# frederik-kofoed-marqversen/quantum_computations

Hardware: AMD Instinct MI355X
Metric: gate_apps_per_sec (higher is better)
Workload: dtype f64; 1 GPU; 28-qubit complex128 state vector (28 qubits = 4 GiB per GPU), depth-100 random 1+2-qubit gates (BASELINE.json configs[1], seed 100); n_qubits=28

## Files before the change

### quantum_computations_amd/build.py

```python
from __future__ import annotations

import os
import shutil
import subprocess
import sys
from pathlib import Path

PKG_DIR = Path(__file__).resolve().parent
REPO_ROOT = PKG_DIR.parent
CSRC = PKG_DIR / "csrc"
LIB_PATH = PKG_DIR / "libqsv.so"
SOURCES = ["qsv_api.hip", "qsv_kernels.hip", "qsv_qudit.hip", "qsv_gemm.hip", "qsv_decomp.hip", "qsv_circuit.hip",
           "qsv_phase_space.hip", "qsv_sampling.hip", "qsv_canonical.hip"]
HEADERS = [CSRC / "qsv_internal.h", CSRC / "qsv_linalg.h", CSRC / "qsv_plan.h", CSRC / "qsv_layout.h", CSRC / "qsv_pauli_plan.h",
           CSRC / "qsv_pauli_rotation_plan.h", REPO_ROOT / "include" / "qsv.h"]
ARCH = "gfx950"


def hipcc() -> str:
    for cand in (os.environ.get("HIPCC"), shutil.which("hipcc"), "/opt/rocm/bin/hipcc"):
        if cand and Path(cand).exists():
            return cand
    raise RuntimeError("hipcc not found: libqsv.so needs the ROCm toolchain (there is no CPU fallback)")


def _stale(target: Path, deps: list[Path]) -> bool:
    if not target.exists():
        return True
    t = target.stat().st_mtime
    return any(d.stat().st_mtime > t for d in deps)


def build_lib(force: bool = False, verbose: bool = False) -> Path:
    objs = []
    build_dir = PKG_DIR / "build"
    build_dir.mkdir(exist_ok=True)
    flags = [f"--offload-arch={ARCH}", "-O3", "-std=c++17", "-fPIC", "-Wall", "-Wno-unused-function",
             f"-I{REPO_ROOT / 'include'}", f"-I{CSRC}"]
    for name in SOURCES:
        src = CSRC / name
        obj = build_dir / (name + ".o")
        if force or _stale(obj, [src] + HEADERS):
            cmd = [hipcc(), *flags, "-c", str(src), "-o", str(obj)]
            if verbose:
                print(" ".join(cmd), flush=True)
            subprocess.run(cmd, check=True)
        objs.append(obj)
    if force or _stale(LIB_PATH, objs):
        cmd = [hipcc(), f"--offload-arch={ARCH}", "-shared", "-fPIC", "-o", str(LIB_PATH), *map(str, objs), "-ldl"]
        if verbose:
            print(" ".join(cmd), flush=True)
        subprocess.run(cmd, check=True)
    return LIB_PATH


if __name__ == "__main__":
    path = build_lib(force="--force" in sys.argv, verbose=True)
    print(path)
```

### quantum_computations_amd/csrc/qsv_kernels.hip

```cpp

#include "qsv_internal.h"
#include "qsv_layout.h"
#include "qsv_plan.h"

#include <algorithm>
#include <array>
#include <cstdlib>
#include <cstring>
#include <type_traits>
#include <vector>

using namespace qsv_layout;
static_assert(LANE_BITS == QSV_LANE_BITS && MAX_K == QSV_MAX_K && BLOCK == QSV_BLOCK, "qsv_layout.h and qsv_internal.h agree");

namespace {

struct cplx {
    double re, im;
};

__device__ __forceinline__ amp_t cmul(cplx m, amp_t a) {
    amp_t r;
    r.x = m.re * a.x - m.im * a.y;
    r.y = m.re * a.y + m.im * a.x;
    return r;
}

__device__ __forceinline__ amp_t cmul_diag(cplx d, amp_t a) {
    amp_t r;
    r.x = fma(a.x, d.re, -(a.y * d.im));
    r.y = fma(a.x, d.im, a.y * d.re);
    return r;
}

__device__ __forceinline__ amp_t cfma(cplx m, amp_t a, amp_t acc) {
    amp_t r;
    r.x = fma(m.re, a.x, fma(-m.im, a.y, acc.x));
    r.y = fma(m.re, a.y, fma(m.im, a.x, acc.y));
    return r;
}

template <bool NT>
__device__ __forceinline__ amp_t ld(const amp_t *p) {
    if constexpr (NT)
        return __builtin_nontemporal_load(p);
    else
        return *p;
}

template <bool NT>
__device__ __forceinline__ void st(amp_t *p, amp_t v) {
    if constexpr (NT)
        __builtin_nontemporal_store(v, p);
    else
        *p = v;
}

__device__ __forceinline__ amp_t shfl_xor_amp(amp_t v, int lane_mask) {
    amp_t r;
    r.x = __shfl_xor(v.x, lane_mask, 64);
    r.y = __shfl_xor(v.y, lane_mask, 64);
    return r;
}

__device__ __forceinline__ uint64_t insert_zero(uint64_t w, int p) {
    const uint64_t low = w & ((1ull << p) - 1ull);
    return ((w >> p) << (p + 1)) | low;
}

template <class Args>
__device__ __forceinline__ uint64_t deposit(uint64_t w, const Args &g) {
    for (int j = 0; j < g.nins; ++j) w = insert_zero(w, static_cast<int>(g.pos[j]));
    return w | g.or_mask;
}

template <int KH, int KL, int U, bool NT>
__device__ __forceinline__ void dense_body(amp_t *__restrict__ a, const GateArgs &g) {
    constexpr int NH = 1 << KH, NL = 1 << KL, D = NH * NL;
    const int lane = threadIdx.x & 63;
    const bool lane_ok = (static_cast<uint32_t>(lane) & g.lane_ctrl) == g.lane_ctrl;

    int l = 0;
#pragma unroll
    for (int j = 0; j < KL; ++j) l |= ((lane >> g.lbit[j]) & 1) << j;

    cplx coef[NH][NH][NL];
#pragma unroll
    for (int h = 0; h < NH; ++h)
#pragma unroll
        for (int hp = 0; hp < NH; ++hp)
#pragma unroll
            for (int x = 0; x < NL; ++x) {
// ... 2188 lines not shown
    return rc ? rc : qsvk_stage_done(st, staged);
}

int qsvk_sequence_tile(qsv_state *st, int k, const int *bits, int n_gates, const int *arity, const int *legs,
                       const double *mats) {
    if (k < 1 || k > 6 || n_gates < 1 || n_gates > SEQ_MAX_GATES || st->n < TILE_SEQ_BITS) return QSV_UNHANDLED_KQ;
    const TileCut cut = cut_tile_passes(st->n, k, bits, n_gates, arity, legs, mats);
    if (cut.status == TileCut::UNHANDLED) return QSV_UNHANDLED_KQ;
    if (cut.status == TileCut::LEG_OUTSIDE) return qsv_fail(QSV_EINVAL, "gate sequence: leg outside the block");
    if (cut.status == TileCut::LEGS_EQUAL) return qsv_fail(QSV_EINVAL, "gate sequence: legs outside the block");
    const std::vector<int> &tile_bits = cut.tile_bits;
    const std::vector<uint64_t> off = offsets(std::vector<int>(tile_bits.begin() + 6, tile_bits.end()));
    const size_t gates_bytes = qsv_pad16(sizeof(SeqGate) * cut.rec.size()), passes_bytes = qsv_pad16(sizeof(TilePass) * cut.passes.size());
    std::vector<char> image(gates_bytes + passes_bytes, 0);
    std::memcpy(image.data(), cut.rec.data(), sizeof(SeqGate) * cut.rec.size());
    std::memcpy(image.data() + gates_bytes, cut.passes.data(), sizeof(TilePass) * cut.passes.size());
    StageRef staged;
    int rc = qsvk_stage(st, image.data(), image.size(), off.data(), sizeof(uint64_t) * off.size(), &staged);
    if (rc) return rc;
    const SeqGate *dev_g = reinterpret_cast<const SeqGate *>(staged.dev);
    const TilePass *dev_p = reinterpret_cast<const TilePass *>(staged.dev + gates_bytes);
    const uint64_t *dev_off = reinterpret_cast<const uint64_t *>(staged.dev + qsv_pad16(image.size()));
    TileSeqArgs ta;
    std::memset(&ta, 0, sizeof(ta));
    ta.g = with_enumeration<BigArgs>(enumeration(st->amps >> TILE_SEQ_BITS, tile_bits));
    for (int j = 0; j < 6; ++j) ta.lane_bit[j] = static_cast<uint32_t>(tile_bits[j]);
    ta.g.regions = regions_or(st, 8);
    const bool nt = st->nontemporal != 0;
    const size_t lds = sizeof(amp_t) << TILE_SEQ_BITS;
    static bool raised = false;
    if (!raised) {
        QSV_HIP(hipFuncSetAttribute(reinterpret_cast<const void *>(k_seq_tile<true>), hipFuncAttributeMaxDynamicSharedMemorySize,
                                    static_cast<int>(lds)));
        QSV_HIP(hipFuncSetAttribute(reinterpret_cast<const void *>(k_seq_tile<false>), hipFuncAttributeMaxDynamicSharedMemorySize,
                                    static_cast<int>(lds)));
        raised = true;
    }
    snprintf(st->last_kernel, sizeof(st->last_kernel), "k_seq_tile<%s>", nt ? "true" : "false");
    const int n_passes = static_cast<int>(cut.passes.size());
    st->last_passes = n_passes;
    rc = launch_ranges(ta.g, DISPATCH_TILES, [&](uint64_t tiles) {
        const dim3 gd(static_cast<unsigned>(tiles)), bd(TILE_SEQ_THREADS);
        with_bool(nt, [&](auto NT) { hipLaunchKernelGGL(k_seq_tile<NT.value>, gd, bd, lds, st->stream, st->data, ta, dev_g, dev_p, n_passes, dev_off); });
    });
    return rc ? rc : qsvk_stage_done(st, staged);
}

constexpr int PASS_TILE = 1 << qsv_plan::TILE_BITS, PASS_ROWS = PASS_TILE / 64, PASS_THREADS = 256;
constexpr int PASS_ROWS_PER_WAVE = PASS_ROWS / (PASS_THREADS / 64);
static_assert(PASS_TILE == PASS_THREADS << qsv_plan::REG_BITS, "one thread per setting of the tile bits outside the registers");

struct PassArgs {
    BigArgs g;
    uint64_t row_off[PASS_ROWS];
};

template <int FORM>
__device__ __forceinline__ constexpr int pass_col(int r, int j) {
    return FORM == 0 ? j : FORM == 1 ? (j ^ r) : (((j & 1) << 1) | ((r & 1) ^ (j >> 1)));
}

struct PassCtl {
    uint32_t rc;
    bool sel;
    bool ok;
};

__device__ __forceinline__ void pass_put(amp_t &x, amp_t y, const PassCtl &ct) {
    if (ct.sel) {
        x.x = ct.ok ? y.x : x.x;
        x.y = ct.ok ? y.y : x.y;
    } else {
        x = y;
    }
}

template <int D, int FORM, int P0, int P1>
__device__ __forceinline__ void pass_dense(amp_t (&x)[16], const double *__restrict__ m, const PassCtl &ct) {
    constexpr int TARGETS = (1 << P0) | (D == 4 ? (1 << P1) : 0);
#pragma unroll
    for (int b = 0; b < 16; ++b) {
        if (b & TARGETS) continue;
        if ((b & ct.rc) != ct.rc) continue;
        int idx[D];
#pragma unroll
        for (int c = 0; c < D; ++c) idx[c] = b | ((c & 1) << P0) | (D == 4 ? ((c >> 1) << P1) : 0);
        amp_t y[D];
#pragma unroll
        for (int r = 0; r < D; ++r) {
            amp_t acc = {0.0, 0.0};
#pragma unroll
            for (int j = 0; j < D; ++j) {
                const int c = pass_col<FORM>(r, j);
                acc = cfma(cplx{m[2 * (r * D + c)], m[2 * (r * D + c) + 1]}, x[idx[c]], acc);
            }
            y[r] = acc;
        }
#pragma unroll
        for (int r = 0; r < D; ++r) pass_put(x[idx[r]], y[r], ct);
    }
}

template <int PA, int PB>
__device__ __forceinline__ void pass_pair(amp_t (&x)[16], const PassCtl &ct) {
#pragma unroll
    for (int b = 0; b < 16; ++b) {
        if (b & ((1 << PA) | (1 << PB))) continue;
        if ((b & ct.rc) != ct.rc) continue;
        const amp_t u = x[b | (1 << PA)], v = x[b | (1 << PB)];
        pass_put(x[b | (1 << PA)], v, ct);
        pass_put(x[b | (1 << PB)], u, ct);
    }
}

template <class Sel>
__device__ __forceinline__ void pass_diag(amp_t (&x)[16], const cplx (&d)[4], const PassCtl &ct, Sel sel) {
#pragma unroll
    for (int c = 0; c < 16; ++c) {
        if ((c & ct.rc) != ct.rc) continue;
        pass_put(x[c], cmul_diag(d[sel(c)], x[c]), ct);
    }
}

__device__ __forceinline__ cplx pass_pick(bool s, cplx one, cplx zero) {
    return cplx{s ? one.re : zero.re, s ? one.im : zero.im};
}

__device__ __forceinline__ void pass_gate16(amp_t (&x)[16], const PassGate &pg, uint32_t g0) {
    const double *__restrict__ m = pg.m;
    const PassCtl ct = {pg.rc, pg.tc != 0, (g0 & pg.tc) == pg.tc};
#define QSV_PASS_D4(FORM, P0, P1) case (FORM) * 16 + (P0) * 4 + (P1): pass_dense<4, (FORM) - PASS_D4, P0, P1>(x, m, ct); break;
#define QSV_PASS_D4_BOTH(FORM, LO, HI) QSV_PASS_D4(FORM, LO, HI) QSV_PASS_D4(FORM, HI, LO)
    switch (pg.form * 16 + pg.code) {
        case PASS_D2 * 16 + 0: pass_dense<2, 0, 0, 0>(x, m, ct); break;
        case PASS_D2 * 16 + 1: pass_dense<2, 0, 1, 0>(x, m, ct); break;
        case PASS_D2 * 16 + 2: pass_dense<2, 0, 2, 0>(x, m, ct); break;
        case PASS_D2 * 16 + 3: pass_dense<2, 0, 3, 0>(x, m, ct); break;
        case PASS_D2X * 16 + 0: pass_dense<2, 1, 0, 0>(x, m, ct); break;
        case PASS_D2X * 16 + 1: pass_dense<2, 1, 1, 0>(x, m, ct); break;
        case PASS_D2X * 16 + 2: pass_dense<2, 1, 2, 0>(x, m, ct); break;
        case PASS_D2X * 16 + 3: pass_dense<2, 1, 3, 0>(x, m, ct); break;
        QSV_PASS_D4_BOTH(PASS_D4, 0, 1) QSV_PASS_D4_BOTH(PASS_D4, 0, 2) QSV_PASS_D4_BOTH(PASS_D4, 0, 3)
        QSV_PASS_D4_BOTH(PASS_D4, 1, 2) QSV_PASS_D4_BOTH(PASS_D4, 1, 3) QSV_PASS_D4_BOTH(PASS_D4, 2, 3)
        QSV_PASS_D4_BOTH(PASS_D4X, 0, 1) QSV_PASS_D4_BOTH(PASS_D4X, 0, 2) QSV_PASS_D4_BOTH(PASS_D4X, 0, 3)
        QSV_PASS_D4_BOTH(PASS_D4X, 1, 2) QSV_PASS_D4_BOTH(PASS_D4X, 1, 3) QSV_PASS_D4_BOTH(PASS_D4X, 2, 3)
        QSV_PASS_D4(PASS_D4HL, 0, 1) QSV_PASS_D4(PASS_D4HL, 0, 2) QSV_PASS_D4(PASS_D4HL, 0, 3)
        QSV_PASS_D4(PASS_D4HL, 1, 2) QSV_PASS_D4(PASS_D4HL, 1, 3) QSV_PASS_D4(PASS_D4HL, 2, 3)
        case PASS_PAIR * 16 + 0 * 4 + 1: pass_pair<0, 1>(x, ct); break;
        case PASS_PAIR * 16 + 0 * 4 + 2: pass_pair<0, 2>(x, ct); break;
        case PASS_PAIR * 16 + 0 * 4 + 3: pass_pair<0, 3>(x, ct); break;
        case PASS_PAIR * 16 + 1 * 4 + 2: pass_pair<1, 2>(x, ct); break;
        case PASS_PAIR * 16 + 1 * 4 + 3: pass_pair<1, 3>(x, ct); break;
        case PASS_PAIR * 16 + 2 * 4 + 3: pass_pair<2, 3>(x, ct); break;
        case PASS_DIAG_T * 16: {
            const bool s0 = (g0 >> pg.tz0) & 1, s1 = (g0 >> pg.tz1) & 1;
            const cplx d[4] = {pass_pick(s0, pass_pick(s1, cplx{m[6], m[7]}, cplx{m[4], m[5]}),
                                         pass_pick(s1, cplx{m[2], m[3]}, cplx{m[0], m[1]})), {}, {}, {}};
            pass_diag(x, d, ct, [](int) { return 0; });
            break;
        }
#define QSV_PASS_R1(P) case PASS_DIAG_R1 * 16 + (P): { \
            const cplx d[4] = {{m[0], m[1]}, {m[2], m[3]}, {}, {}}; \
            pass_diag(x, d, ct, [](int c) { return (c >> (P)) & 1; }); break; }
        QSV_PASS_R1(0) QSV_PASS_R1(1) QSV_PASS_R1(2) QSV_PASS_R1(3)
#define QSV_PASS_R2(P0, P1) case PASS_DIAG_R2 * 16 + (P0) * 4 + (P1): { \
            const cplx d[4] = {{m[0], m[1]}, {m[2], m[3]}, {m[4], m[5]}, {m[6], m[7]}}; \
            pass_diag(x, d, ct, [](int c) { return (((c >> (P0)) & 1) << 1) | ((c >> (P1)) & 1); }); break; }
        QSV_PASS_R2(0, 1) QSV_PASS_R2(0, 2) QSV_PASS_R2(0, 3) QSV_PASS_R2(1, 2) QSV_PASS_R2(1, 3) QSV_PASS_R2(2, 3)
#define QSV_PASS_M(P) case PASS_DIAG_M * 16 + (P): { \
            const bool s = (g0 >> pg.tz0) & 1; \
            const cplx d[4] = {pass_pick(s, cplx{m[2], m[3]}, cplx{m[0], m[1]}), pass_pick(s, cplx{m[6], m[7]}, cplx{m[4], m[5]}), {}, {}}; \
            pass_diag(x, d, ct, [](int c) { return (c >> (P)) & 1; }); break; }
        QSV_PASS_M(0) QSV_PASS_M(1) QSV_PASS_M(2) QSV_PASS_M(3)
        default: break;
    }
#undef QSV_PASS_D4
#undef QSV_PASS_D4_BOTH
#undef QSV_PASS_R1
#undef QSV_PASS_R2
#undef QSV_PASS_M
}

template <bool NT>
__global__ __launch_bounds__(PASS_THREADS) void k_pass_tile(amp_t *__restrict__ a, const PassArgs pa,
                                                            const PassGate *__restrict__ gates, int n_gates,
                                                            const PassGroup *__restrict__ groups, int n_groups) {
    __shared__ amp_t tile[PASS_TILE];
    const BigArgs &g = pa.g;
    const int lane = threadIdx.x & 63;
    const int q = __builtin_amdgcn_readfirstlane(threadIdx.x >> 6);
    constexpr int RPW = PASS_ROWS_PER_WAVE;
    const uint64_t tile_id = (g.regions > 1 && gridDim.x % g.regions == 0)
                                 ? (blockIdx.x % g.regions) * (gridDim.x / g.regions) + blockIdx.x / g.regions
                                 : blockIdx.x;
    const uint64_t base = deposit(g.w0 + tile_id, g);
    uint64_t active = 0;
    for (int i = 0; i < n_gates; ++i)
        if ((base & gates[i].omask) == gates[i].omask) active |= 1ull << i;
    if (!active) return;
#if defined(__HIP_DEVICE_COMPILE__)
#pragma unroll
    for (int i = 0; i < RPW; ++i)
        __builtin_amdgcn_global_load_lds(a + base + pa.row_off[q * RPW + i] + lane, tile + (q * RPW + i) * 64, 16, 0, NT ? 2 : 0);
#endif
    __syncthreads();
#pragma unroll 1
    for (int p = 0; p < n_groups; ++p) {
        const PassGroup &gr = groups[p];
        if (!(active & gr.gates)) continue;
        const int q0 = gr.q[0], q1 = gr.q[1], q2 = gr.q[2], q3 = gr.q[3];
        uint32_t g0 = threadIdx.x;
        g0 = static_cast<uint32_t>(insert_zero(g0, q0));
        g0 = static_cast<uint32_t>(insert_zero(g0, q1));
        g0 = static_cast<uint32_t>(insert_zero(g0, q2));
        g0 = static_cast<uint32_t>(insert_zero(g0, q3));
        amp_t x[16];
#pragma unroll
        for (int c = 0; c < 16; ++c)
            x[c] = tile[g0 | ((c & 1) << q0) | (((c >> 1) & 1) << q1) | (((c >> 2) & 1) << q2) | (((c >> 3) & 1) << q3)];
#pragma unroll 1
        for (int i = gr.first; i < gr.first + gr.count; ++i)
            if ((active >> i) & 1) pass_gate16(x, gates[i], g0);
#pragma unroll
        for (int c = 0; c < 16; ++c)
            tile[g0 | ((c & 1) << q0) | (((c >> 1) & 1) << q1) | (((c >> 2) & 1) << q2) | (((c >> 3) & 1) << q3)] = x[c];
        __syncthreads();
    }
#pragma unroll
    for (int i = 0; i < RPW; ++i) st<NT>(a + base + pa.row_off[q * RPW + i] + lane, tile[(q * RPW + i) * 64 + lane]);
}

bool qsvk_op_exact(const QsvOp &op) {
    if (op.kind == QSV_OP_PAIR) return true;
    auto unit = [](double re, double im) { return im == 0.0 && (re == 1.0 || re == -1.0); };
    if (op.kind == QSV_OP_PHASE) return unit(op.m[0], op.m[1]);
    if (op.kind == QSV_OP_DIAG) {
        for (int i = 0; i < (1 << op.k); ++i)
            if (!unit(op.m[2 * i], op.m[2 * i + 1])) return false;
        return true;
    }
    const int D = 1 << op.k;
    int per_col[4] = {0, 0, 0, 0};
    for (int r = 0; r < D; ++r) {
        int nz = 0;
        for (int c = 0; c < D; ++c) {
            const double re = op.m[2 * (r * D + c)], im = op.m[2 * (r * D + c) + 1];
            if (re == 0.0 && im == 0.0) continue;
            if (!unit(re, im)) return false;
            ++nz;
            ++per_col[c];
        }
        if (nz != 1) return false;
    }
    for (int c = 0; c < D; ++c)
        if (per_col[c] != 1) return false;
    return true;
}

int qsvk_run_op(qsv_state *st, const QsvOp &op) {
    switch (op.kind) {
        case QSV_OP_DENSE: return qsvk_dense(st, op.k, op.bits, op.nctrl, op.cbits, op.m);
        case QSV_OP_PAIR: return qsvk_pair_exchange(st, op.bits[0], op.bits[1]);
        case QSV_OP_DIAG: return qsvk_diag(st, op.k, op.bits, op.nctrl, op.cbits, op.m);
        case QSV_OP_PHASE: return qsvk_phase(st, op.nctrl, op.cbits, op.m[0], op.m[1]);
        default: return qsv_fail(QSV_EINVAL, "internal: unknown queued gate kind");
    }
}

int qsvk_pass(qsv_state *st, const QsvOp *const *ops, int count, uint64_t tile_high) {
    const uint64_t low = (1ull << QSV_LANE_BITS) - 1;
    if (count < 1 || count > qsv_plan::MAX_PASS_GATES || st->n < qsv_plan::TILE_BITS || (tile_high & low) ||
        __builtin_popcountll(tile_high) != qsv_plan::HIGH_BITS || (tile_high >> st->n))
        return qsv_fail(QSV_EINVAL, "internal: malformed gate pass");
    const PassRecords pr = pass_records(ops, count, tile_high, st->amps);
    if (pr.status == PassRecords::TARGET_OUTSIDE_TILE) return qsv_fail(QSV_EINVAL, "internal: gate target outside its pass's tile");
    if (pr.status == PassRecords::TARGET_OUTSIDE_GROUP) return qsv_fail(QSV_EINVAL, "internal: gate target outside its group's register bits");
    StageRef staged;
    int rc = qsvk_stage(st, pr.rec.data(), sizeof(PassGate) * pr.rec.size(), pr.grp.data(), sizeof(PassGroup) * pr.grp.size(), &staged);
    if (rc) return rc;
    const PassGate *dev_g = reinterpret_cast<const PassGate *>(staged.dev);
    const PassGroup *dev_p = reinterpret_cast<const PassGroup *>(staged.dev + qsv_pad16(sizeof(PassGate) * pr.rec.size()));
    const int n_groups = static_cast<int>(pr.grp.size());
    const std::vector<int> tile_bits(pr.tile_bits, pr.tile_bits + qsv_plan::TILE_BITS);
    PassArgs pa;
    std::memset(&pa, 0, sizeof(pa));
    pa.g = with_enumeration<BigArgs>(enumeration(st->amps >> qsv_plan::TILE_BITS, tile_bits));
    const std::vector<uint64_t> row_off = offsets(std::vector<int>(tile_bits.begin() + QSV_LANE_BITS, tile_bits.end()));
    std::copy(row_off.begin(), row_off.end(), pa.row_off);
    pa.g.regions = regions_or(st, 8);
    const bool nt = st->nontemporal != 0;
    snprintf(st->last_kernel, sizeof(st->last_kernel), "k_pass_tile<%s>", nt ? "true" : "false");
    rc = launch_ranges(pa.g, DISPATCH_TILES, [&](uint64_t tiles) {
        const dim3 gd(static_cast<unsigned>(tiles)), bd(PASS_THREADS);
        with_bool(nt, [&](auto NT) { hipLaunchKernelGGL(k_pass_tile<NT.value>, gd, bd, 0, st->stream, st->data, pa, dev_g, count, dev_p, n_groups); });
    });
    return rc ? rc : qsvk_stage_done(st, staged);
}

static int launch_dense_mfma(qsv_state *st, int k, const int *bits, const double *m_user, const FormChoice &f) {
    const int D = 1 << k;
    std::vector<int> sorted(bits, bits + k);
    std::sort(sorted.begin(), sorted.end());
    const std::vector<uint64_t> off = offsets(sorted);
    const std::vector<double> m = matrix(f.realm ? MAT_COLUMNS_REAL : MAT_COLUMNS, D, m_user, user_index(k, bits, sorted.data()).data());
    StageRef staged;
    int rc = qsvk_stage(st, m.data(), sizeof(double) * m.size(), off.data(), sizeof(uint64_t) * D, &staged);
    if (rc) return rc;
    const double *dev_m = reinterpret_cast<const double *>(staged.dev);
    const uint64_t *dev_off = reinterpret_cast<const uint64_t *>(staged.dev + qsv_pad16(sizeof(double) * m.size()));
    const Mfma6Args g = with_enumeration<Mfma6Args>(enumeration(st->amps >> k, sorted));
    const bool nt = st->nontemporal != 0;
    const size_t lds = sizeof(double) * m.size() + sizeof(uint64_t) * D;
    int cus = 256;
    (void)hipDeviceGetAttribute(&cus, hipDeviceAttributeMultiprocessorCount, st->device);
    const uint64_t wave_tiles = g.W / 16;
    const unsigned grid = static_cast<unsigned>(std::min<uint64_t>((wave_tiles + 3) / 4, ((k == 6 && !f.realm) ? 2ull : 3ull) * cus));
    snprintf(st->last_kernel, sizeof(st->last_kernel), "k_dense_mfma<%d, %s, %s%s>", k, nt ? "true" : "false",
             f.realm ? "true" : "false", f.m3 ? ", true" : "");
    auto launch = [&](auto kernel) -> int {
        QSV_HIP(hipFuncSetAttribute(reinterpret_cast<const void *>(kernel), hipFuncAttributeMaxDynamicSharedMemorySize, static_cast<int>(lds)));
        hipLaunchKernelGGL(kernel, dim3(grid), dim3(QSV_BLOCK), lds, st->stream, st->data, g, dev_m, dev_off);
        return check_launch();
    };
    rc = with_int<5, 6>(k, [&](auto K) { return with_bool(f.realm, [&](auto REAL) { return with_bool(nt, [&](auto NT) {
        if constexpr (!REAL.value) {
            if (f.m3) return launch(k_dense_mfma<K.value, NT.value, false, true>);
        }
        return launch(k_dense_mfma<K.value, NT.value, REAL.value>);
    }); }); });
    return rc ? rc : qsvk_stage_done(st, staged);
}

int qsvk_generic(qsv_state *st, int k, const int *bits, const double *m_user) {
    if (k < 1 || k > QSV_MAX_K) return qsv_fail(QSV_EINVAL, "generic gate: k must be in 1..6");
    const FormChoice f = choose_form(st->n, st->amps, k, bits, is_real(1 << k, m_user),
                                     FormOptions{st->kq_variant, st->complex_product, mtile_default()});
    if (f.form == FORM_MFMA) return launch_dense_mfma(st, k, bits, m_user, f);
    if (f.form != FORM_GATHER) return launch_dense_big(st, k, bits, m_user, f);
    const size_t bytes = sizeof(double) * 2ull << (2 * k);
    StageRef staged;
    int rc = qsvk_stage(st, m_user, bytes, nullptr, 0, &staged);
    if (rc) return rc;
    const double *dev_m = reinterpret_cast<const double *>(staged.dev);
    GenericArgs g;
    std::memset(&g, 0, sizeof(g));
    g.K = k;
    g.W = st->amps >> k;
// ... 664 lines not shown
```

### quantum_computations_amd/csrc/qsv_layout.h

```cpp
#pragma once

#include <stdint.h>
#include <string.h>

#include <algorithm>
#include <array>
#include <vector>

#include "qsv_plan.h"

namespace qsv_layout {

constexpr int LANE_BITS = 6;
constexpr int LINE_BITS = 3;
constexpr int MAX_K = 6;
constexpr int BLOCK = 256;


struct BigArgs {
    uint64_t W;
    int32_t nins;
    uint32_t pos[2 * MAX_K];
    uint64_t or_mask;
    uint64_t w0;
    uint32_t regions;
    int32_t lbit[MAX_K];
};

struct LdsArgs {
    uint64_t W;
    int32_t nins;
    uint32_t pos[2 * MAX_K];
    uint64_t or_mask;
    uint64_t w0;
    uint32_t regions;
    uint32_t amask;
    int32_t abit[3], aE[3];
    int32_t na;
    uint32_t bdep[8];
    uint32_t bmask;
};

struct SmallGate {
    double m[32];
    uint64_t off[4];
};

struct SeqGate {
    int32_t code;
    int32_t pad[3];
    double m[32];
};
constexpr int SEQ_MAX_GATES = 48;

struct TilePass {
    int32_t first, count;
    int32_t q[4];
    int32_t pad[2];
};
constexpr int TILE_SEQ_BITS = 12, TILE_SEQ_ROWS = 1 << (TILE_SEQ_BITS - 6), TILE_SEQ_THREADS = 256, TILE_SEQ_MAX_PASSES = 24;

enum {
    PASS_D2 = 0, PASS_D2X = 1, PASS_D4 = 2, PASS_D4X = 3, PASS_D4HL = 4,
    PASS_PAIR = 5,
    PASS_DIAG_T = 6, PASS_DIAG_R1 = 7, PASS_DIAG_R2 = 8, PASS_DIAG_M = 9
};
struct PassGate {
    int32_t form;
    int32_t code;
    uint32_t rc;
    uint32_t tc;
    int32_t tz0, tz1;
    uint64_t omask;
    double m[32];
};
struct PassGroup {
    int32_t first, count;
    int32_t q[4];
    uint64_t gates;
};

enum { OP_DENSE = 0, OP_PAIR = 1, OP_DIAG = 2, OP_PHASE = 3 };
constexpr int OP_MAX_CTRL = 40;
struct Op {
    int kind = OP_DENSE;
    int k = 0;
    int bits[2] = {-1, -1};
    int nctrl = 0;
    int cbits[OP_MAX_CTRL] = {};
    double m[32] = {};
};

struct Split {
    std::vector<int> high, low, standin;
    bool enough = true;
    int KB = 0;
};
inline Split split_targets(int k, const int *bits, int n) {
    Split s;
    for (int j = 0; j < k; ++j) (bits[j] >= LANE_BITS ? s.high : s.low).push_back(bits[j]);
    std::sort(s.low.begin(), s.low.end());
    for (int b = LANE_BITS; b < n && s.standin.size() < s.low.size(); ++b)
        if (std::find(s.high.begin(), s.high.end(), b) == s.high.end()) s.standin.push_back(b);
    s.enough = s.standin.size() == s.low.size();
    for (int b : s.low) s.KB += b < LINE_BITS;
    return s;
}
inline Split untransposed(int k, const int *bits) {
    Split s;
    s.high.assign(bits, bits + k);
    return s;
}

inline std::vector<uint64_t> offsets(const std::vector<int> &addr_bit) {
    std::vector<uint64_t> off(1ull << addr_bit.size(), 0);
    for (size_t c = 0; c < off.size(); ++c)
        for (size_t i = 0; i < addr_bit.size(); ++i)
            if ((c >> i) & 1) off[c] |= 1ull << addr_bit[i];
    return off;
}

inline std::vector<int> kernel_bits(const Split &s) {
    std::vector<int> kb(s.low);
    kb.insert(kb.end(), s.high.begin(), s.high.end());
    return kb;
}
inline std::vector<int> address_bits(const Split &s, bool a_in_place) {
    std::vector<int> ab;
// ... 252 lines not shown
};
inline std::vector<Range> dispatch_ranges(uint64_t W, uint64_t limit) {
    std::vector<Range> out;
    for (uint64_t w0 = 0; w0 < W; w0 += limit) out.push_back(Range{w0, std::min(limit, W - w0)});
    return out;
}

enum Form { FORM_GATHER , FORM_MFMA, FORM_MTILE5, FORM_TILE, FORM_LDS, FORM_BIG };
struct FormChoice {
    Form form = FORM_GATHER;
    bool transposed = false;
    bool realm = false;
    bool m3 = false;
};
struct FormOptions {
    int kq_variant = 0;
    int complex_product = 0;
    bool mtile = false;
};
inline FormChoice choose_form(int n, uint64_t amps, int k, const int *bits, bool real_matrix, const FormOptions &o) {
    FormChoice f;
    const bool mfma_ok = n >= k && (amps >> k) >= 16;
    if (mfma_ok && ((k == 6 && o.kq_variant == 0) || (k == 5 && o.kq_variant == 5))) {
        f.form = FORM_MFMA;
        f.realm = real_matrix;
        f.m3 = !real_matrix && o.complex_product != 4;
        return f;
    }
    if (k < 3 || n < k) return f;
    const Split s = split_targets(k, bits, n);
    bool all_from_bit3 = true;
    for (int j = 0; j < k; ++j) all_from_bit3 = all_from_bit3 && bits[j] >= LINE_BITS;
    const bool fits = (amps >> k) >= 64 && (amps >> k) % 64 == 0;
    const bool tile_ok = k <= 5 && all_from_bit3 && fits;
    const bool use_mtile = tile_ok && k == 5 && !real_matrix && o.complex_product != 4 &&
                           (o.kq_variant == 6 || (o.kq_variant == 0 && o.mtile));
    const bool use_tile = use_mtile || (tile_ok && (o.kq_variant == 4 || (o.kq_variant == 0 && (k <= 4 || real_matrix))));
    f.transposed = !s.low.empty() && s.enough && o.kq_variant != 2 && !use_tile;
    const int KL = f.transposed ? static_cast<int>(s.low.size()) : 0;
    const bool use_lds = !use_tile && fits && (k == 6 || o.kq_variant == 3 ||
                                               (o.kq_variant == 0 && k == 5 && (KL > 0 || real_matrix)));
    if (k == 6 && !use_lds) return FormChoice();
    f.form = use_mtile ? FORM_MTILE5 : use_tile ? FORM_TILE : use_lds ? FORM_LDS : FORM_BIG;
    f.realm = (use_lds || use_tile) && real_matrix;
    f.m3 = !use_mtile && k == 5 && !real_matrix && o.complex_product == 3 && (use_tile || use_lds || KL == 0);
    return f;
}

struct PassRecords {
    enum Status { OK, TARGET_OUTSIDE_TILE, TARGET_OUTSIDE_GROUP } status = OK;
    int tile_bits[qsv_plan::TILE_BITS] = {};
    std::vector<PassGate> rec;
    std::vector<PassGroup> grp;
};
inline PassRecords pass_records(const Op *const *ops, int count, uint64_t tile_high, uint64_t amps) {
    PassRecords out;
    int local_of[64];
    for (int b = 0; b < 64; ++b) {
        local_of[b] = qsv_plan::tile_index(b, tile_high);
        if (local_of[b] >= 0) out.tile_bits[local_of[b]] = b;
    }
    std::vector<PassGate> &rec = out.rec;
    rec.resize(count);
    std::vector<std::array<int, 2>> leg(count, std::array<int, 2>{-1, -1});
    std::vector<uint32_t> cmask(count, 0), need(count, 0);
    for (int i = 0; i < count; ++i) {
        const Op &op = *ops[i];
        PassGate &pg = rec[i];
        memset(&pg, 0, sizeof(pg));
        uint64_t ctrl = 0;
        for (int c = 0; c < op.nctrl; ++c) ctrl |= 1ull << op.cbits[c];
        const qsv_plan::ControlMasks cm = qsv_plan::control_masks(ctrl, tile_high);
        cmask[i] = cm.inside;
        pg.omask = cm.outside;
        for (int j = 0; j < op.k; ++j)
            if (local_of[op.bits[j]] < 0) return out.status = PassRecords::TARGET_OUTSIDE_TILE, out;
        if (op.kind == OP_DIAG || op.kind == OP_PHASE) {
            pg.form = PASS_DIAG_T;
            if (op.kind == OP_PHASE) {
                for (int e = 0; e < 4; ++e) {
                    pg.m[2 * e] = op.m[0];
                    pg.m[2 * e + 1] = op.m[1];
                }
            } else {
                leg[i][0] = local_of[op.bits[0]];
                if (op.k == 2) leg[i][1] = local_of[op.bits[1]];
                memcpy(pg.m, op.m, sizeof(double) * (2u << op.k));
            }
            continue;
        }
        if (op.kind == OP_PAIR) {
            pg.form = PASS_PAIR;
            leg[i] = {local_of[op.bits[0]], local_of[op.bits[1]]};
            need[i] = (1u << leg[i][0]) | (1u << leg[i][1]);
            continue;
        }
        const int k = op.k;
        int kb[2] = {op.bits[0], op.bits[1]};
        if (tile12_takes(amps, k, op.bits, op.nctrl, op.cbits)) {
            pg.form = k == 1 ? PASS_D2 : PASS_D4;
        } else {
            int nl = 0, nh = 0;
            for (int j = 0; j < k; ++j) nl += op.bits[j] < LANE_BITS;
            for (int j = 0, l = 0; j < k; ++j) kb[op.bits[j] < LANE_BITS ? l++ : nl + nh++] = op.bits[j];
            pg.form = nl == 0 ? (k == 1 ? PASS_D2 : PASS_D4) : nh == 0 ? (k == 1 ? PASS_D2X : PASS_D4X) : PASS_D4HL;
        }
        write_matrix(MAT_COMPLEX, 1 << k, op.m, user_index(k, op.bits, kb).data(), pg.m);
        for (int i2 = 0; i2 < k; ++i2) {
            leg[i][i2] = local_of[kb[i2]];
            need[i] |= 1u << leg[i][i2];
        }
    }
    const std::vector<qsv_plan::Group> cut = qsv_plan::cut_groups(need);
    out.grp.resize(cut.size());
    for (size_t p = 0; p < cut.size(); ++p) {
        PassGroup &gr = out.grp[p];
        memset(&gr, 0, sizeof(gr));
        gr.first = cut[p].first;
        gr.count = cut[p].count;
        int reg_of[qsv_plan::TILE_BITS];
        for (int t = 0; t < qsv_plan::TILE_BITS; ++t) reg_of[t] = -1;
        for (int j = 0; j < qsv_plan::REG_BITS; ++j) {
            gr.q[j] = cut[p].reg[j];
            reg_of[gr.q[j]] = j;
        }
        for (int i = gr.first; i < gr.first + gr.count; ++i) {
            PassGate &pg = rec[i];
            gr.gates |= 1ull << i;
            for (int t = 0; t < qsv_plan::TILE_BITS; ++t)
                if ((cmask[i] >> t) & 1) {
                    if (reg_of[t] >= 0) pg.rc |= 1u << reg_of[t];
                    else pg.tc |= 1u << t;
                }
            const int l0 = leg[i][0], l1 = leg[i][1];
            if (pg.form == PASS_DIAG_T) {
                const int r0 = l0 >= 0 ? reg_of[l0] : -1, r1 = l1 >= 0 ? reg_of[l1] : -1;
                auto swap_d1_d2 = [&pg]() {
                    std::swap(pg.m[2], pg.m[4]);
                    std::swap(pg.m[3], pg.m[5]);
                };
                if (l0 < 0) {
                    pg.tz0 = pg.tz1 = 0;
                } else if (l1 < 0) {
                    if (r0 >= 0) {
                        pg.form = PASS_DIAG_R1;
                        pg.code = r0;
                    } else {
                        pg.m[6] = pg.m[2];
                        pg.m[7] = pg.m[3];
                        pg.tz0 = pg.tz1 = l0;
                    }
                } else if (r0 >= 0 && r1 >= 0) {
                    pg.form = PASS_DIAG_R2;
                    if (r0 > r1) swap_d1_d2();
                    pg.code = std::min(r0, r1) * 4 + std::max(r0, r1);
                } else if (r0 >= 0 || r1 >= 0) {
                    pg.form = PASS_DIAG_M;
                    if (r0 < 0) swap_d1_d2();
                    pg.code = r0 >= 0 ? r0 : r1;
                    pg.tz0 = r0 >= 0 ? l1 : l0;
                } else {
                    pg.tz0 = l0;
                    pg.tz1 = l1;
                }
                continue;
            }
            const int r0 = reg_of[l0], r1 = l1 >= 0 ? reg_of[l1] : 0;
            if (r0 < 0 || r1 < 0) return out.status = PassRecords::TARGET_OUTSIDE_GROUP, out;
            if (pg.form == PASS_PAIR) pg.code = std::min(r0, r1) * 4 + std::max(r0, r1);
            else if (pg.form == PASS_D2 || pg.form == PASS_D2X) pg.code = r0;
            else pg.code = r0 * 4 + r1;
        }
    }
    return out;
}

}
```

Baseline: 4286 gate-apps/s.

## Specialize pass-tile gate control paths and issue tile loads before mask scan

Adds a compile-time control mode (none, register, thread) to each pass gate so uncontrolled gates skip the per-element select logic. The dense kernels now interleave accumulation across rows. Row offsets are computed from bit positions instead of being read from a kernel-arg table. When any gate applies to every tile, the global-to-LDS load is issued before the active-gate mask scan, overlapping the scan with memory traffic; the omask array is read in batches of eight. It also adds an LLVM flag to skip uniform-region structurization and a build-time probe that fails if the flag is unsupported. This adds template variants and so more code size.

```diff
diff --git a/quantum_computations_amd/build.py b/quantum_computations_amd/build.py
--- a/quantum_computations_amd/build.py
+++ b/quantum_computations_amd/build.py
@@ -15,6 +15,16 @@
 HEADERS = [CSRC / "qsv_internal.h", CSRC / "qsv_linalg.h", CSRC / "qsv_plan.h", CSRC / "qsv_layout.h", CSRC / "qsv_pauli_plan.h",
            CSRC / "qsv_pauli_rotation_plan.h", REPO_ROOT / "include" / "qsv.h"]
 ARCH = "gfx950"
+EXTRA_FLAGS = {"qsv_kernels.hip": ["-mllvm", "-structurizecfg-skip-uniform-regions"]}
+
+
+def check_extra_flags() -> None:
+    for name, extra in EXTRA_FLAGS.items():
+        probe = subprocess.run([hipcc(), f"--offload-arch={ARCH}", *extra, "--cuda-device-only", "-x", "hip", "-c", "-",
+                                "-o", os.devnull], input="__global__ void k() {}\n", capture_output=True, text=True)
+        if probe.returncode != 0:
+            raise RuntimeError(f"{hipcc()} does not accept {' '.join(extra)} (needed for {name}, see DESIGN.md section 10):\n"
+                               + probe.stderr[-2000:])
 
 
 def hipcc() -> str:
@@ -32,6 +42,7 @@
 
 
 def build_lib(force: bool = False, verbose: bool = False) -> Path:
+    check_extra_flags()
     objs = []
     build_dir = PKG_DIR / "build"
     build_dir.mkdir(exist_ok=True)
@@ -41,7 +52,7 @@
         src = CSRC / name
         obj = build_dir / (name + ".o")
         if force or _stale(obj, [src] + HEADERS):
-            cmd = [hipcc(), *flags, "-c", str(src), "-o", str(obj)]
+            cmd = [hipcc(), *flags, *EXTRA_FLAGS.get(name, []), "-c", str(src), "-o", str(obj)]
             if verbose:
                 print(" ".join(cmd), flush=True)
             subprocess.run(cmd, check=True)
diff --git a/quantum_computations_amd/csrc/qsv_kernels.hip b/quantum_computations_amd/csrc/qsv_kernels.hip
--- a/quantum_computations_amd/csrc/qsv_kernels.hip
+++ b/quantum_computations_amd/csrc/qsv_kernels.hip
@@ -33,11 +33,20 @@
     return r;
 }
 
+__device__ __forceinline__ amp_t cfma_inner(cplx m, amp_t a, amp_t acc) {
+    amp_t r;
+    r.x = fma(-m.im, a.y, acc.x);
+    r.y = fma(m.im, a.x, acc.y);
+    return r;
+}
+__device__ __forceinline__ amp_t cfma_outer(cplx m, amp_t a, amp_t inner) {
+    amp_t r;
+    r.x = fma(m.re, a.x, inner.x);
+    r.y = fma(m.re, a.y, inner.y);
+    return r;
+}
 __device__ __forceinline__ amp_t cfma(cplx m, amp_t a, amp_t acc) {
-    amp_t r;
-    r.x = fma(m.re, a.x, fma(-m.im, a.y, acc.x));
-    r.y = fma(m.re, a.y, fma(m.im, a.x, acc.y));
-    return r;
+    return cfma_outer(m, a, cfma_inner(m, a, acc));
 }
 
 template <bool NT>
@@ -2332,7 +2341,7 @@
 
 struct PassArgs {
     BigArgs g;
-    uint64_t row_off[PASS_ROWS];
+    uint32_t every_tile;
 };
 
 template <int FORM>
@@ -2342,12 +2351,17 @@
 
 struct PassCtl {
     uint32_t rc;
-    bool sel;
     bool ok;
 };
 
+template <int CTL>
+__device__ __forceinline__ bool pass_skips(int b, const PassCtl &ct) {
+    return CTL != PASS_CTL_NONE && (static_cast<uint32_t>(b) & ct.rc) != ct.rc;
+}
+
+template <int CTL>
 __device__ __forceinline__ void pass_put(amp_t &x, amp_t y, const PassCtl &ct) {
-    if (ct.sel) {
+    if constexpr (CTL == PASS_CTL_THREAD) {
         x.x = ct.ok ? y.x : x.x;
         x.y = ct.ok ? y.y : x.y;
     } else {
@@ -2355,50 +2369,60 @@
     }
 }
 
-template <int D, int FORM, int P0, int P1>
+template <int CTL, int D, int FORM, int P0, int P1>
 __device__ __forceinline__ void pass_dense(amp_t (&x)[16], const double *__restrict__ m, const PassCtl &ct) {
     constexpr int TARGETS = (1 << P0) | (D == 4 ? (1 << P1) : 0);
 #pragma unroll
     for (int b = 0; b < 16; ++b) {
         if (b & TARGETS) continue;
-        if ((b & ct.rc) != ct.rc) continue;
+        if (pass_skips<CTL>(b, ct)) continue;
         int idx[D];
 #pragma unroll
         for (int c = 0; c < D; ++c) idx[c] = b | ((c & 1) << P0) | (D == 4 ? ((c >> 1) << P1) : 0);
+        amp_t acc[D];
+#pragma unroll
+        for (int r = 0; r < D; ++r) acc[r] = amp_t{0.0, 0.0};
+#pragma unroll
+        for (int j = 0; j < D - 1; ++j)
+#pragma unroll
+            for (int r = 0; r < D; ++r) {
+                const int c = pass_col<FORM>(r, j);
+                acc[r] = cfma(cplx{m[2 * (r * D + c)], m[2 * (r * D + c) + 1]}, x[idx[c]], acc[r]);
+            }
+#pragma unroll
+        for (int r = 0; r < D; ++r) {
+            const int c = pass_col<FORM>(r, D - 1);
+            acc[r] = cfma_inner(cplx{m[2 * (r * D + c)], m[2 * (r * D + c) + 1]}, x[idx[c]], acc[r]);
+        }
         amp_t y[D];
 #pragma unroll
         for (int r = 0; r < D; ++r) {
-            amp_t acc = {0.0, 0.0};
-#pragma unroll
-            for (int j = 0; j < D; ++j) {
-                const int c = pass_col<FORM>(r, j);
-                acc = cfma(cplx{m[2 * (r * D + c)], m[2 * (r * D + c) + 1]}, x[idx[c]], acc);
-            }
-            y[r] = acc;
-        }
-#pragma unroll
-        for (int r = 0; r < D; ++r) pass_put(x[idx[r]], y[r], ct);
-    }
-}
-
-template <int PA, int PB>
+            const int c = pass_col<FORM>(r, D - 1);
+            y[r] = cfma_outer(cplx{m[2 * (r * D + c)], m[2 * (r * D + c) + 1]}, x[idx[c]], acc[r]);
+        }
+#pragma unroll
+        for (int r = 0; r < D; ++r) pass_put<CTL>(x[idx[r]], y[r], ct);
+    }
+}
+
+template <int CTL, int PA, int PB>
 __device__ __forceinline__ void pass_pair(amp_t (&x)[16], const PassCtl &ct) {
 #pragma unroll
     for (int b = 0; b < 16; ++b) {
         if (b & ((1 << PA) | (1 << PB))) continue;
-        if ((b & ct.rc) != ct.rc) continue;
+        if (pass_skips<CTL>(b, ct)) continue;
         const amp_t u = x[b | (1 << PA)], v = x[b | (1 << PB)];
-        pass_put(x[b | (1 << PA)], v, ct);
-        pass_put(x[b | (1 << PB)], u, ct);
-    }
-}
-
-template <class Sel>
+        pass_put<CTL>(x[b | (1 << PA)], v, ct);
+        pass_put<CTL>(x[b | (1 << PB)], u, ct);
+    }
+}
+
+template <int CTL, class Sel>
 __device__ __forceinline__ void pass_diag(amp_t (&x)[16], const cplx (&d)[4], const PassCtl &ct, Sel sel) {
 #pragma unroll
     for (int c = 0; c < 16; ++c) {
-        if ((c & ct.rc) != ct.rc) continue;
-        pass_put(x[c], cmul_diag(d[sel(c)], x[c]), ct);
+        if (pass_skips<CTL>(c, ct)) continue;
+        pass_put<CTL>(x[c], cmul_diag(d[sel(c)], x[c]), ct);
     }
 }
 
@@ -2406,51 +2430,52 @@
     return cplx{s ? one.re : zero.re, s ? one.im : zero.im};
 }
 
+template <int CTL>
 __device__ __forceinline__ void pass_gate16(amp_t (&x)[16], const PassGate &pg, uint32_t g0) {
     const double *__restrict__ m = pg.m;
-    const PassCtl ct = {pg.rc, pg.tc != 0, (g0 & pg.tc) == pg.tc};
-#define QSV_PASS_D4(FORM, P0, P1) case (FORM) * 16 + (P0) * 4 + (P1): pass_dense<4, (FORM) - PASS_D4, P0, P1>(x, m, ct); break;
+    const PassCtl ct = {pg.rc, (g0 & pg.tc) == pg.tc};
+#define QSV_PASS_D4(FORM, P0, P1) case (FORM) * 16 + (P0) * 4 + (P1): pass_dense<CTL, 4, (FORM) - PASS_D4, P0, P1>(x, m, ct); break;
 #define QSV_PASS_D4_BOTH(FORM, LO, HI) QSV_PASS_D4(FORM, LO, HI) QSV_PASS_D4(FORM, HI, LO)
     switch (pg.form * 16 + pg.code) {
-        case PASS_D2 * 16 + 0: pass_dense<2, 0, 0, 0>(x, m, ct); break;
-        case PASS_D2 * 16 + 1: pass_dense<2, 0, 1, 0>(x, m, ct); break;
-        case PASS_D2 * 16 + 2: pass_dense<2, 0, 2, 0>(x, m, ct); break;
-        case PASS_D2 * 16 + 3: pass_dense<2, 0, 3, 0>(x, m, ct); break;
-        case PASS_D2X * 16 + 0: pass_dense<2, 1, 0, 0>(x, m, ct); break;
-        case PASS_D2X * 16 + 1: pass_dense<2, 1, 1, 0>(x, m, ct); break;
-        case PASS_D2X * 16 + 2: pass_dense<2, 1, 2, 0>(x, m, ct); break;
-        case PASS_D2X * 16 + 3: pass_dense<2, 1, 3, 0>(x, m, ct); break;
+        case PASS_D2 * 16 + 0: pass_dense<CTL, 2, 0, 0, 0>(x, m, ct); break;
+        case PASS_D2 * 16 + 1: pass_dense<CTL, 2, 0, 1, 0>(x, m, ct); break;
+        case PASS_D2 * 16 + 2: pass_dense<CTL, 2, 0, 2, 0>(x, m, ct); break;
+        case PASS_D2 * 16 + 3: pass_dense<CTL, 2, 0, 3, 0>(x, m, ct); break;
+        case PASS_D2X * 16 + 0: pass_dense<CTL, 2, 1, 0, 0>(x, m, ct); break;
+        case PASS_D2X * 16 + 1: pass_dense<CTL, 2, 1, 1, 0>(x, m, ct); break;
+        case PASS_D2X * 16 + 2: pass_dense<CTL, 2, 1, 2, 0>(x, m, ct); break;
+        case PASS_D2X * 16 + 3: pass_dense<CTL, 2, 1, 3, 0>(x, m, ct); break;
         QSV_PASS_D4_BOTH(PASS_D4, 0, 1) QSV_PASS_D4_BOTH(PASS_D4, 0, 2) QSV_PASS_D4_BOTH(PASS_D4, 0, 3)
         QSV_PASS_D4_BOTH(PASS_D4, 1, 2) QSV_PASS_D4_BOTH(PASS_D4, 1, 3) QSV_PASS_D4_BOTH(PASS_D4, 2, 3)
         QSV_PASS_D4_BOTH(PASS_D4X, 0, 1) QSV_PASS_D4_BOTH(PASS_D4X, 0, 2) QSV_PASS_D4_BOTH(PASS_D4X, 0, 3)
         QSV_PASS_D4_BOTH(PASS_D4X, 1, 2) QSV_PASS_D4_BOTH(PASS_D4X, 1, 3) QSV_PASS_D4_BOTH(PASS_D4X, 2, 3)
         QSV_PASS_D4(PASS_D4HL, 0, 1) QSV_PASS_D4(PASS_D4HL, 0, 2) QSV_PASS_D4(PASS_D4HL, 0, 3)
         QSV_PASS_D4(PASS_D4HL, 1, 2) QSV_PASS_D4(PASS_D4HL, 1, 3) QSV_PASS_D4(PASS_D4HL, 2, 3)
-        case PASS_PAIR * 16 + 0 * 4 + 1: pass_pair<0, 1>(x, ct); break;
-        case PASS_PAIR * 16 + 0 * 4 + 2: pass_pair<0, 2>(x, ct); break;
-        case PASS_PAIR * 16 + 0 * 4 + 3: pass_pair<0, 3>(x, ct); break;
-        case PASS_PAIR * 16 + 1 * 4 + 2: pass_pair<1, 2>(x, ct); break;
-        case PASS_PAIR * 16 + 1 * 4 + 3: pass_pair<1, 3>(x, ct); break;
-        case PASS_PAIR * 16 + 2 * 4 + 3: pass_pair<2, 3>(x, ct); break;
+        case PASS_PAIR * 16 + 0 * 4 + 1: pass_pair<CTL, 0, 1>(x, ct); break;
+        case PASS_PAIR * 16 + 0 * 4 + 2: pass_pair<CTL, 0, 2>(x, ct); break;
+        case PASS_PAIR * 16 + 0 * 4 + 3: pass_pair<CTL, 0, 3>(x, ct); break;
+        case PASS_PAIR * 16 + 1 * 4 + 2: pass_pair<CTL, 1, 2>(x, ct); break;
+        case PASS_PAIR * 16 + 1 * 4 + 3: pass_pair<CTL, 1, 3>(x, ct); break;
+        case PASS_PAIR * 16 + 2 * 4 + 3: pass_pair<CTL, 2, 3>(x, ct); break;
         case PASS_DIAG_T * 16: {
             const bool s0 = (g0 >> pg.tz0) & 1, s1 = (g0 >> pg.tz1) & 1;
             const cplx d[4] = {pass_pick(s0, pass_pick(s1, cplx{m[6], m[7]}, cplx{m[4], m[5]}),
                                          pass_pick(s1, cplx{m[2], m[3]}, cplx{m[0], m[1]})), {}, {}, {}};
-            pass_diag(x, d, ct, [](int) { return 0; });
+            pass_diag<CTL>(x, d, ct, [](int) { return 0; });
             break;
         }
 #define QSV_PASS_R1(P) case PASS_DIAG_R1 * 16 + (P): { \
             const cplx d[4] = {{m[0], m[1]}, {m[2], m[3]}, {}, {}}; \
-            pass_diag(x, d, ct, [](int c) { return (c >> (P)) & 1; }); break; }
+            pass_diag<CTL>(x, d, ct, [](int c) { return (c >> (P)) & 1; }); break; }
         QSV_PASS_R1(0) QSV_PASS_R1(1) QSV_PASS_R1(2) QSV_PASS_R1(3)
 #define QSV_PASS_R2(P0, P1) case PASS_DIAG_R2 * 16 + (P0) * 4 + (P1): { \
             const cplx d[4] = {{m[0], m[1]}, {m[2], m[3]}, {m[4], m[5]}, {m[6], m[7]}}; \
-            pass_diag(x, d, ct, [](int c) { return (((c >> (P0)) & 1) << 1) | ((c >> (P1)) & 1); }); break; }
+            pass_diag<CTL>(x, d, ct, [](int c) { return (((c >> (P0)) & 1) << 1) | ((c >> (P1)) & 1); }); break; }
         QSV_PASS_R2(0, 1) QSV_PASS_R2(0, 2) QSV_PASS_R2(0, 3) QSV_PASS_R2(1, 2) QSV_PASS_R2(1, 3) QSV_PASS_R2(2, 3)
 #define QSV_PASS_M(P) case PASS_DIAG_M * 16 + (P): { \
             const bool s = (g0 >> pg.tz0) & 1; \
             const cplx d[4] = {pass_pick(s, cplx{m[2], m[3]}, cplx{m[0], m[1]}), pass_pick(s, cplx{m[6], m[7]}, cplx{m[4], m[5]}), {}, {}}; \
-            pass_diag(x, d, ct, [](int c) { return (c >> (P)) & 1; }); break; }
+            pass_diag<CTL>(x, d, ct, [](int c) { return (c >> (P)) & 1; }); break; }
         QSV_PASS_M(0) QSV_PASS_M(1) QSV_PASS_M(2) QSV_PASS_M(3)
         default: break;
     }
@@ -2461,10 +2486,19 @@
 #undef QSV_PASS_M
 }
 
+__device__ __forceinline__ void pass_gate16(amp_t (&x)[16], const PassGate &pg, uint32_t g0) {
+    switch (pg.ctl) {
+        case PASS_CTL_NONE: pass_gate16<PASS_CTL_NONE>(x, pg, g0); break;
+        case PASS_CTL_REG: pass_gate16<PASS_CTL_REG>(x, pg, g0); break;
+        default: pass_gate16<PASS_CTL_THREAD>(x, pg, g0); break;
+    }
+}
+
 template <bool NT>
 __global__ __launch_bounds__(PASS_THREADS) void k_pass_tile(amp_t *__restrict__ a, const PassArgs pa,
                                                             const PassGate *__restrict__ gates, int n_gates,
-                                                            const PassGroup *__restrict__ groups, int n_groups) {
+                                                            const PassGroup *__restrict__ groups, int n_groups,
+                                                            const uint64_t *__restrict__ omask) {
     __shared__ amp_t tile[PASS_TILE];
     const BigArgs &g = pa.g;
     const int lane = threadIdx.x & 63;
@@ -2473,16 +2507,40 @@
     const uint64_t tile_id = (g.regions > 1 && gridDim.x % g.regions == 0)
                                  ? (blockIdx.x % g.regions) * (gridDim.x / g.regions) + blockIdx.x / g.regions
                                  : blockIdx.x;
-    const uint64_t base = deposit(g.w0 + tile_id, g);
+    uint64_t base = g.w0 + tile_id;
+#pragma unroll
+    for (int j = 0; j < qsv_plan::TILE_BITS; ++j) base = insert_zero(base, static_cast<int>(g.pos[j]));
+    base |= g.or_mask;
+    static_assert(RPW == 16 && PASS_ROWS == 64, "four row bits from i, two from the wave number");
+    uint64_t row0 = base + (static_cast<uint64_t>(q & 1) << g.pos[10]) + (static_cast<uint64_t>(q >> 1) << g.pos[11]);
+    auto row = [&](int i) {
+        uint64_t r = row0;
+#pragma unroll
+        for (int j = 0; j < 4; ++j)
+            if ((i >> j) & 1) r += 1ull << g.pos[6 + j];
+        return r;
+    };
+    auto request_tile = [&]() {
+#if defined(__HIP_DEVICE_COMPILE__)
+#pragma unroll
+        for (int i = 0; i < RPW; ++i)
+            __builtin_amdgcn_global_load_lds(a + row(i) + lane, tile + (q * RPW + i) * 64, 16, 0, NT ? 2 : 0);
+#endif
+    };
+    if (pa.every_tile) request_tile();
     uint64_t active = 0;
-    for (int i = 0; i < n_gates; ++i)
-        if ((base & gates[i].omask) == gates[i].omask) active |= 1ull << i;
-    if (!active) return;
-#if defined(__HIP_DEVICE_COMPILE__)
-#pragma unroll
-    for (int i = 0; i < RPW; ++i)
-        __builtin_amdgcn_global_load_lds(a + base + pa.row_off[q * RPW + i] + lane, tile + (q * RPW + i) * 64, 16, 0, NT ? 2 : 0);
-#endif
+    for (int i0 = 0; i0 < n_gates; i0 += 8) {
+        uint64_t om[8];
+#pragma unroll
+        for (int j = 0; j < 8; ++j) om[j] = omask[i0 + j];
+#pragma unroll
+        for (int j = 0; j < 8; ++j) active |= static_cast<uint64_t>((base & om[j]) == om[j]) << (i0 + j);
+    }
+    active &= ~0ull >> (64 - n_gates);
+    if (!pa.every_tile) {
+        if (!active) return;
+        request_tile();
+    }
     __syncthreads();
 #pragma unroll 1
     for (int p = 0; p < n_groups; ++p) {
@@ -2506,8 +2564,11 @@
             tile[g0 | ((c & 1) << q0) | (((c >> 1) & 1) << q1) | (((c >> 2) & 1) << q2) | (((c >> 3) & 1) << q3)] = x[c];
         __syncthreads();
     }
-#pragma unroll
-    for (int i = 0; i < RPW; ++i) st<NT>(a + base + pa.row_off[q * RPW + i] + lane, tile[(q * RPW + i) * 64 + lane]);
+#if defined(__HIP_DEVICE_COMPILE__)
+    asm volatile("" : "+s"(row0));
+#endif
+#pragma unroll
+    for (int i = 0; i < RPW; ++i) st<NT>(a + row(i) + lane, tile[(q * RPW + i) * 64 + lane]);
 }
 
 bool qsvk_op_exact(const QsvOp &op) {
@@ -2555,24 +2616,28 @@
     const PassRecords pr = pass_records(ops, count, tile_high, st->amps);
     if (pr.status == PassRecords::TARGET_OUTSIDE_TILE) return qsv_fail(QSV_EINVAL, "internal: gate target outside its pass's tile");
     if (pr.status == PassRecords::TARGET_OUTSIDE_GROUP) return qsv_fail(QSV_EINVAL, "internal: gate target outside its group's register bits");
+    const size_t grp_bytes = sizeof(PassGroup) * pr.grp.size(), omask_count = (pr.omask.size() + 7) / 8 * 8;
+    std::vector<char> tail(grp_bytes + sizeof(uint64_t) * omask_count, 0);
+    std::memcpy(tail.data(), pr.grp.data(), grp_bytes);
+    std::memcpy(tail.data() + grp_bytes, pr.omask.data(), sizeof(uint64_t) * pr.omask.size());
     StageRef staged;
-    int rc = qsvk_stage(st, pr.rec.data(), sizeof(PassGate) * pr.rec.size(), pr.grp.data(), sizeof(PassGroup) * pr.grp.size(), &staged);
+    int rc = qsvk_stage(st, pr.rec.data(), sizeof(PassGate) * pr.rec.size(), tail.data(), tail.size(), &staged);
     if (rc) return rc;
     const PassGate *dev_g = reinterpret_cast<const PassGate *>(staged.dev);
     const PassGroup *dev_p = reinterpret_cast<const PassGroup *>(staged.dev + qsv_pad16(sizeof(PassGate) * pr.rec.size()));
+    const uint64_t *dev_o = reinterpret_cast<const uint64_t *>(reinterpret_cast<const char *>(dev_p) + grp_bytes);
     const int n_groups = static_cast<int>(pr.grp.size());
     const std::vector<int> tile_bits(pr.tile_bits, pr.tile_bits + qsv_plan::TILE_BITS);
     PassArgs pa;
     std::memset(&pa, 0, sizeof(pa));
     pa.g = with_enumeration<BigArgs>(enumeration(st->amps >> qsv_plan::TILE_BITS, tile_bits));
-    const std::vector<uint64_t> row_off = offsets(std::vector<int>(tile_bits.begin() + QSV_LANE_BITS, tile_bits.end()));
-    std::copy(row_off.begin(), row_off.end(), pa.row_off);
     pa.g.regions = regions_or(st, 8);
+    pa.every_tile = pr.every_tile ? 1u : 0u;
     const bool nt = st->nontemporal != 0;
     snprintf(st->last_kernel, sizeof(st->last_kernel), "k_pass_tile<%s>", nt ? "true" : "false");
     rc = launch_ranges(pa.g, DISPATCH_TILES, [&](uint64_t tiles) {
         const dim3 gd(static_cast<unsigned>(tiles)), bd(PASS_THREADS);
-        with_bool(nt, [&](auto NT) { hipLaunchKernelGGL(k_pass_tile<NT.value>, gd, bd, 0, st->stream, st->data, pa, dev_g, count, dev_p, n_groups); });
+        with_bool(nt, [&](auto NT) { hipLaunchKernelGGL(k_pass_tile<NT.value>, gd, bd, 0, st->stream, st->data, pa, dev_g, count, dev_p, n_groups, dev_o); });
     });
     return rc ? rc : qsvk_stage_done(st, staged);
 }
diff --git a/quantum_computations_amd/csrc/qsv_layout.h b/quantum_computations_amd/csrc/qsv_layout.h
--- a/quantum_computations_amd/csrc/qsv_layout.h
+++ b/quantum_computations_amd/csrc/qsv_layout.h
@@ -65,15 +65,19 @@
     PASS_PAIR = 5,
     PASS_DIAG_T = 6, PASS_DIAG_R1 = 7, PASS_DIAG_R2 = 8, PASS_DIAG_M = 9
 };
+enum { PASS_CTL_NONE = 0, PASS_CTL_REG = 1, PASS_CTL_THREAD = 2 };
 struct PassGate {
     int32_t form;
     int32_t code;
     uint32_t rc;
     uint32_t tc;
     int32_t tz0, tz1;
+    int32_t ctl;
+    int32_t pad0;
     uint64_t omask;
     double m[32];
 };
+static_assert(sizeof(PassGate) == 40 + 32 * sizeof(double), "no padding but pad0");
 struct PassGroup {
     int32_t first, count;
     int32_t q[4];
@@ -432,6 +436,8 @@
     int tile_bits[qsv_plan::TILE_BITS] = {};
     std::vector<PassGate> rec;
     std::vector<PassGroup> grp;
+    std::vector<uint64_t> omask;
+    bool every_tile = false;
 };
 inline PassRecords pass_records(const Op *const *ops, int count, uint64_t tile_high, uint64_t amps) {
     PassRecords out;
@@ -453,6 +459,8 @@
         const qsv_plan::ControlMasks cm = qsv_plan::control_masks(ctrl, tile_high);
         cmask[i] = cm.inside;
         pg.omask = cm.outside;
+        out.omask.push_back(pg.omask);
+        out.every_tile = out.every_tile || pg.omask == 0;
         for (int j = 0; j < op.k; ++j)
             if (local_of[op.bits[j]] < 0) return out.status = PassRecords::TARGET_OUTSIDE_TILE, out;
         if (op.kind == OP_DIAG || op.kind == OP_PHASE) {
@@ -512,6 +520,7 @@
                     if (reg_of[t] >= 0) pg.rc |= 1u << reg_of[t];
                     else pg.tc |= 1u << t;
                 }
+            pg.ctl = pg.tc ? PASS_CTL_THREAD : pg.rc ? PASS_CTL_REG : PASS_CTL_NONE;
             const int l0 = leg[i][0], l1 = leg[i][1];
             if (pg.form == PASS_DIAG_T) {
                 const int r0 = l0 >= 0 ? reg_of[l0] : -1, r1 = l1 >= 0 ? reg_of[l1] : -1;
```

Measured after the change: 5205 gate-apps/s, median of 6. 21.4% higher.
